# emanuele-artioli/elvis

Hardware: AMD Instinct MI355X
Metric: restored 1080p frames/sec, SinSR 4x path (ELVIS v2 Downsample) (higher is better)
Workload: dtype f16; 1 GPU; 30-frame 1920x1080 synthetic clip per GPU, ELVIS v2 Downsample (SinSR 4x), block 8, levels 0-3, weights seed 0 (random init), quantize=True; frames_per_gpu=30, parallelism=single GPU, gn_fused_into_conv=True, frames_per_invocation=15

## Files before the change

### elvis_amd/_lib.py

```python
from __future__ import annotations

import ctypes as C
import os
import threading
from typing import Optional

HERE = os.path.dirname(os.path.abspath(__file__))
LIBPATH = os.environ.get("ELVIS_AMD_LIB") or os.path.join(HERE, "lib", "libelvis_amd.so")

F32, F16 = 0, 1
ROUND_CV2, ROUND_HALF_UP = 0, 1
SSIM_LUMA, SSIM_CHANNELS = 0, 1
SSIM_REFLECT, SSIM_VALID = 0, 1
SSIM_PAD_AUTO = -1

_lock = threading.Lock()
_lib: Optional[C.CDLL] = None

vp, i32, f32, i64, f64 = C.c_void_p, C.c_int, C.c_float, C.c_longlong, C.c_double


class ConvDesc(C.Structure):
    _fields_ = [(n, C.c_int) for n in (
        "dtype", "n", "h", "w", "cin", "cin_pitch", "cin2", "cin2_pitch", "cout", "cout_pitch",
        "ksize", "stride", "pad_before", "upsample", "ho", "wo", "act", "prologue", "subpixel")]


SIGNATURES = {
    "elvis_abi_version": [],
    "elvis_last_error": [],
    "elvis_last_launch": [],
    "elvis_recompose_u8": [vp, vp, vp, vp, vp, i32, i32, i32, i32, i32, i32, i32, i32, i32, vp],
    "elvis_area_downscale_u8": [vp, vp, i32, i32, i32, i32, i32, i32, vp],
    "elvis_blend_u8": [vp, vp, vp, vp, i32, i32, i32, i32, i32, i32, i32, f32, vp],
    "elvis_select_levels_u8": [vp, vp, i32, vp, vp, i32, i32, i32, i32, i32, i32, i32, vp],
    "elvis_tile_accumulate_f32": [vp, vp, vp, vp, vp, vp, i32, i32, i32, i32, i32, i32, i32, f32, vp],
    "elvis_tile_normalize_u8": [vp, vp, vp, i32, i32, i32, vp],
    "elvis_sse_u8": [vp, vp, vp, vp, vp, i32, i32, i32, i32, vp],
    "elvis_block_ssim_u8": [vp, vp, vp, vp, i32, i32, i32, i32, i32, vp],
    "elvis_mask_bbox_u8": [vp, vp, i32, i32, i32, vp],
    "elvis_apply_mask_u8": [vp, vp, vp, i32, i32, i32, i32, i32, vp],
    "elvis_ssim_workspace_bytes": [i32, i32, i32, i32],
    "elvis_ssim_mean_f64": [vp, vp, vp, vp, vp, vp, vp, i32, i32, i32, i32, i32, i32, f64, f64, f64, i32, f64, vp],
    "elvis_u8_to_float": [vp, vp, i32, i32, i32, i32, i32, f32, f32, i32, i32, vp],
    "elvis_float_to_u8": [vp, i32, vp, vp, i32, i32, i32, i32, f32, f32, i32, i32, vp],
    "elvis_conv_packed_weight_bytes": [C.POINTER(ConvDesc)],
    "elvis_conv_pack_weights": [C.POINTER(ConvDesc), vp, vp, vp],
    "elvis_conv2d": [C.POINTER(ConvDesc), vp, vp, vp, vp, vp, i32, vp, vp, vp, vp, vp],
    "elvis_conv_stats_tiles": [C.POINTER(ConvDesc)],
    "elvis_conv_kernel_name": [C.POINTER(ConvDesc), C.c_char_p, C.c_size_t],
    "elvis_conv_kernel_name_for_call": [C.POINTER(ConvDesc), i32, i32, C.c_char_p, C.c_size_t],
    "elvis_conv_x3_eligible": [C.POINTER(ConvDesc)],
    "elvis_conv_debug_set": [C.c_char_p, i32],
    "elvis_gn_partials_to_sums": [vp, i32, i32, i32, vp, i32, i32, vp],
    "elvis_groupnorm_workspace_floats": [i32, i32, i32, i32],
    "elvis_groupnorm_sums": [vp, i32, i32, i32, i32, i32, vp, i32, i32, vp, vp],
    "elvis_groupnorm_affine": [vp, vp, vp, vp, vp, vp, vp, i32, i32, i32, i32, f32, vp],
    "elvis_affine_act": [vp, vp, i32, i32, i32, i32, i32, i32, vp, vp, i32, vp],
    "elvis_layernorm": [vp, vp, i32, i64, i32, i32, i32, vp, vp, f32, vp],
    "elvis_swin_packed_bytes": [i32, i32, i32],
    "elvis_swin_pack_weights": [vp, vp, vp, i32, i32, i32, vp],
    "elvis_swin_mlp": [vp, vp, vp, vp, vp, vp, vp, i64, i32, i32, i32, i32, f32, vp],
    "elvis_swin_ln_linear": [vp, vp, vp, vp, vp, vp, i64, i32, i32, i32, i32, f32, vp],
    "elvis_swin_pack_proj_mlp": [vp, vp, vp, vp, i32, i32, vp],
    "elvis_swin_proj_mlp": [vp, vp, vp, vp, vp, vp, vp, vp, vp, i64, i32, i32, i32, i32, i32, f32, vp],
    "elvis_window_attention": [vp, vp, i32, i32, i32, i32, i32, i32, i32, i32, i32, i32, vp, f32, vp],
    "elvis_bicubic_upsample": [vp, vp, i32, i32, i32, i32, i32, i32, i32, i32, vp],
    "elvis_vq_nearest": [vp, vp, vp, i32, i64, i32, i32, i32, vp, i32, vp],
    "elvis_pad_reflect_axpy": [vp, vp, i32, i32, i32, i32, i32, i32, i32, i32, i32, i32, f32, vp, f32, vp],
    "elvis_crop_copy": [vp, vp, i32, i32, i32, i32, i32, i32, i32, i32, i32, vp],
    "elvis_convert_act": [vp, i32, vp, i32, i64, i32, vp],
    "elvis_degrade_downsample_u8": [vp, vp, vp, i32, i32, i32, i32, i32, i32, i32, vp],
    "elvis_degrade_gaussian_u8": [vp, vp, vp, i32, i32, i32, i32, i32, i32, i32, f32, f32, f32, vp],
    "elvis_degrade_dct_u8": [vp, vp, vp, vp, vp, i32, i32, i32, i32, i32, i32, i32, vp],
    "elvis_degrade_scale_u8": [vp, vp, vp, i32, i32, i32, i32, i32, i32, i32, vp, vp, vp, i32, vp],
    "elvis_degrade_gaussian_fx_u8": [vp, vp, vp, i32, i32, i32, i32, i32, i32, i32, i32, i32, i32, vp],
    "elvis_rgb_to_i420_u8": [vp, vp, i32, i32, i32, i32, vp],
    "elvis_i420_to_rgb_u8": [vp, vp, i32, i32, i32, i32, vp],
    "elvis_classical_lanczos_u8": [vp, vp, vp, i32, i32, i32, i32, i32, i32, i32, vp, vp],
    "elvis_classical_unsharp_u8": [vp, vp, vp, i32, i32, i32, i32, i32, i32, i32, i32, vp, vp, i32, vp],
    "elvis_temporal_blend_u8": [vp, vp, i32, i64, f64, f64, vp],
# ... 19 lines not shown
    "elvis_rrdb_packed_weight_bytes": [i32, i32],
    "elvis_rrdb_pack_weights": [vp, i32, i32, i32, i32, vp],
    "elvis_rrdb_conv3x3": [vp, i32, vp, vp, vp, i32, i32, vp, i32, vp, i32, i32, i32, i32, i32, i32, i32, i32, f32, f32, i32, i32, vp],
    "elvis_rrdb_input_u8": [vp, vp, i32, i32, i32, i32, i32, vp],
    "elvis_dcnv2": [vp, vp, vp, vp, vp, i32, i32, i32, i32, i32, i32, i32, i32, i32, i32, i32, i32, vp],
    "elvis_temporal_stack": [vp, vp, i32, i32, i32, i32, i32, i32, i32, i32, vp],
    "elvis_plane_merge": [vp, vp, vp, i32, i32, i32, i32, i32, i32, vp],
}


def lib() -> C.CDLL:
    global _lib
    if _lib is not None:
        return _lib
    with _lock:
        if _lib is not None:
            return _lib
        if not os.path.exists(LIBPATH):
            raise RuntimeError(
                f"libelvis_amd.so not found at {LIBPATH}. Build it with `python -m elvis_amd._build` "
                "(needs hipcc). There is no CPU fallback for the restoration path.")
        import torch
        try:
            handle = C.CDLL(LIBPATH)
        except OSError as exc:
            raise RuntimeError(f"failed to load {LIBPATH}: {exc}") from exc
        for name, argtypes in SIGNATURES.items():
            fn = getattr(handle, name)
            fn.argtypes = argtypes
            fn.restype = C.c_int
        handle.elvis_last_error.restype = C.c_char_p
        handle.elvis_last_launch.restype = C.c_char_p
        handle.elvis_conv_packed_weight_bytes.restype = C.c_size_t
        handle.elvis_groupnorm_workspace_floats.restype = C.c_size_t
        handle.elvis_swin_packed_bytes.restype = C.c_size_t
        handle.elvis_ssim_workspace_bytes.restype = C.c_size_t
        handle.elvis_inpaint_workspace_bytes.restype = C.c_size_t
        handle.elvis_lpips_distance_workspace_bytes.restype = C.c_size_t
        handle.elvis_rrdb_packed_weight_bytes.restype = C.c_size_t
        if handle.elvis_abi_version() != 1:
            raise RuntimeError("libelvis_amd.so ABI version mismatch")
        _lib = handle
    return _lib


def check(rc: int, device=None) -> None:
    if rc == 0:
        return
    msg = lib().elvis_last_error().decode("utf-8", "replace")
    if rc == -1:
        raise ValueError(msg)
    label = str(device) if device is not None else "unknown device"
    raise RuntimeError(f"elvis_amd kernel failed on {label}: {msg}")


def ptr(t) -> int:
    return 0 if t is None else t.data_ptr()


def stream_handle(device=None) -> int:
    import torch
    return torch.cuda.current_stream(device).cuda_stream


def require_gpu(device) -> None:
    import torch
# ... 24 lines not shown
```

### elvis_amd/csrc/conv.hip

```cpp
#include "conv_kernels.inc"
#include "conv_ws.inc"
#include <string.h>

__attribute__((visibility("hidden"))) int elvis_conv_launch_f32_(const void* conv_args, int halo, int tco, int id, hipStream_t stream, void* query);
__attribute__((visibility("hidden"))) int elvis_conv_pack_x3p_(const float* w_oihw, void* packed, int cout, int ctot, int nkc, int n_co_tiles,
                                                              int tco, int taps, hipStream_t stream);

#include <atomic>
static std::atomic<int> g_no_halo{0};
static bool no_halo() { return g_no_halo.load(std::memory_order_relaxed) > 0; }
extern "C" int elvis_conv_debug_set(const char* key, int value) {
    ELVIS_REQUIRE(key, "elvis_conv_debug_set: null key");
    if (!strcmp(key, "no_halo")) { g_no_halo.store(value, std::memory_order_relaxed); return ELVIS_OK; }
    ELVIS_REQUIRE(false, "elvis_conv_debug_set: unknown key '%s'", key);
}

static void conv_geom(const elvis_conv_desc* d, int* nkc1, int* nkc, int* co_pad) {
    int kc = kc_of(d);
    *nkc1 = (d->cin + kc - 1) / kc;
    *nkc = *nkc1 + (d->cin2 > 0 ? (d->cin2 + kc - 1) / kc : 0);
    TileCfg t = choose_tile(d->cout);
    *co_pad = ((d->cout + t.tco - 1) / t.tco) * t.tco;
}

extern "C" size_t elvis_conv_packed_weight_bytes(const elvis_conv_desc* d) {
    if (!d || d->cin <= 0 || d->cout <= 0) return 0;
    int nkc1, nkc, co_pad;
    conv_geom(d, &nkc1, &nkc, &co_pad);
    return (size_t)d->ksize * d->ksize * nkc * co_pad * (x3_planar_fmt(d) ? 128 : 64);
}

extern "C" int elvis_conv_pack_weights(const elvis_conv_desc* d, const float* w_oihw, void* packed,
                                       elvis_stream_t stream) {
    int rc = validate(d);
    if (rc) return rc;
    ELVIS_REQUIRE(w_oihw && packed, "elvis_conv_pack_weights: null pointer");
    int nkc1, nkc, co_pad;
    conv_geom(d, &nkc1, &nkc, &co_pad);
    if (x3_planar_fmt(d)) {
        const int tco = choose_tile(d->cout).tco;
        return elvis_conv_pack_x3p_(w_oihw, packed, d->cout, d->cin + d->cin2, nkc, co_pad / tco, tco, d->ksize * d->ksize, (hipStream_t)stream);
    }
    int KC = kc_elems(d->dtype);
    long long total = (long long)d->ksize * d->ksize * nkc * co_pad * KC;
    int grid = (int)((total + 255) / 256);
    int ctot = d->cin + d->cin2;
// ... 71 lines not shown
    int rc = conv_walk(d, path, a, nullptr, &pick);
    if (rc) return rc;
    a.tiles_x = ((subpix ? d->w : d->wo) + HALO_TX - 1) / HALO_TX;
    a.tiles_y = pick.ty > 0 ? ((subpix ? d->h : d->ho) + pick.ty - 1) / pick.ty : 0;
    a.strip = HALO_STRIP < a.tiles_x ? HALO_STRIP : 0;
    a.strip_full = a.strip > 0 ? a.tiles_x / a.strip : 0;
    return ELVIS_OK;
}

extern "C" int elvis_conv_stats_tiles(const elvis_conv_desc* d) {
    if (!d || !halo_eligible(d)) return 0;
    ConvArgs a{};
    ConvPick pick{};
    if (conv_plan(d, ConvPath::HALO, a, pick)) return 0;
    return d->n * a.tiles_y * a.tiles_x;
}

extern "C" int elvis_conv_kernel_name_for_call(const elvis_conv_desc* d, int has_residual, int has_stats, char* buf, size_t n) {
    int rc = validate(d);
    if (rc) return rc;
    ELVIS_REQUIRE(buf && n > 0, "elvis_conv_kernel_name: null buffer");
    ConvArgs a{};
    ConvPick pick{};
    rc = conv_plan(d, conv_path(d, has_residual != 0, has_stats != 0), a, pick);
    if (rc) return rc;
    snprintf(buf, n, "%s", pick.name);
    return ELVIS_OK;
}

extern "C" int elvis_conv_kernel_name(const elvis_conv_desc* d, char* buf, size_t n) {
    return elvis_conv_kernel_name_for_call(d, 0, 0, buf, n);
}

extern "C" int elvis_conv2d(const elvis_conv_desc* d, const void* x, const void* x2, const void* w_packed,
                            const float* bias, const void* residual, int residual_pitch, const float* pa,
                            const float* pb, void* out, float* stats, elvis_stream_t stream) {
    int rc = validate(d);
    if (rc) return rc;
    ELVIS_REQUIRE(x && w_packed && out, "elvis_conv2d: null pointer");
    ELVIS_REQUIRE(d->cin2 == 0 || x2, "elvis_conv2d: cin2 > 0 but x2 is null");
    ELVIS_REQUIRE(!d->prologue || (pa && pb), "elvis_conv2d: prologue requested without pa/pb");
    ELVIS_REQUIRE(d->dtype != ELVIS_F32X3 || x3_eligible(d),
                  "elvis_conv2d: this shape has no compensated-f16 kernel (elvis_conv_x3_eligible): run it as ELVIS_F32");
    ELVIS_REQUIRE(!residual || residual_pitch >= d->cout, "elvis_conv2d: bad residual pitch");
    ELVIS_REQUIRE(((uintptr_t)x | (uintptr_t)(x2 ? x2 : x) | (uintptr_t)w_packed | (uintptr_t)out) % 16 == 0,
                  "elvis_conv2d: pointers must be 16-byte aligned");
    const ConvPath path = conv_path(d, residual != nullptr, stats != nullptr);
    ELVIS_REQUIRE(path != ConvPath::IGEMM || !stats, "elvis_conv2d: fused statistics need a 3x3/stride-1 conv with cout >= 64 (query elvis_conv_stats_tiles)");
    ELVIS_REQUIRE(path == ConvPath::IGEMM || (long long)d->n * d->h * d->w < 0x7fffffffLL, "conv: input too large for 32-bit pixel indices");
    ConvArgs a{};
    ConvPick pick{};
    rc = conv_plan(d, path, a, pick);
    if (rc) return rc;
    a.x = x; a.x2 = x2; a.w = w_packed; a.bias = bias; a.res = residual; a.pa = pa; a.pb = pb; a.out = out;
    a.res_pitch = residual_pitch; a.stats = stats;
    return conv_walk(d, path, a, (hipStream_t)stream, nullptr);
}
```

### elvis_amd/csrc/conv_kernels.inc

```
#pragma once
#include "common.h"

#ifndef ELVIS_CONV_HOOKS
#define ELVIS_STAGE(x) x
#define ELVIS_STAGE_W(x) x
#define ELVIS_STAGE_H(x) x
#define ELVIS_SETPRIO(x)
#define ELVIS_BARRIER() __syncthreads()
#define ELVIS_HOOK_SKIP_STORE(tv)
#define ELVIS_HOOK_STAMP_BEGIN
#define ELVIS_HOOK_STAMP_LOOP
#define ELVIS_HOOK_STAMP_EPILOGUE
#define ELVIS_HOOK_STAMP_END
#endif

namespace {

struct ConvArgs {
    const void* x;
    const void* x2;
    const void* w;
    const float* bias;
    const void* res;
    const float* pa;
    const float* pb;
    void* out;
    int n, h, w_in;
    int cin, cin_pitch, cin2, cin2_pitch;
    int cout, cout_pitch, res_pitch;
    int ksize, stride, pad, upsample;
    int ho, wo;
    int act, prologue;
    int nkc;
    int nkc1;
    int co_pad;
    long long M;
    int n_co_tiles;
    long long n_px_tiles;
    int two, tall;
    float* stats;
    int tiles_x, tiles_y;
    int sub, par_a, par_b;
    int ostr, pad2y, pad2x;
    int s2d, istr, nkc_c, wfull;
    int strip;
    int strip_full;
    int x3;
};

struct ConvPick {
    const char* name;
    int ty;
    int set(const char* name_, int ty_) { name = name_; ty = ty_; return ELVIS_OK; }
};
constexpr const char* tf(bool b) { return b ? "true" : "false"; }

template <typename T> struct Frag;
template <> struct Frag<half_t> { typedef half8 type; };
template <> struct Frag<float> { typedef float4v type; };

__device__ __forceinline__ void mma_tile(float4v& acc, const half8& a, const half8& b) {
    acc = __builtin_amdgcn_mfma_f32_16x16x32_f16(a, b, acc, 0, 0, 0);
}
__device__ __forceinline__ void mma_tile(float4v& acc, const float4v& a, const float4v& b) {
    acc = __builtin_amdgcn_mfma_f32_16x16x4f32(a[0], b[0], acc, 0, 0, 0);
    acc = __builtin_amdgcn_mfma_f32_16x16x4f32(a[1], b[1], acc, 0, 0, 0);
    acc = __builtin_amdgcn_mfma_f32_16x16x4f32(a[2], b[2], acc, 0, 0, 0);
    acc = __builtin_amdgcn_mfma_f32_16x16x4f32(a[3], b[3], acc, 0, 0, 0);
}

__device__ __forceinline__ unsigned x3_pair(float v) {
    const half_t h = (half_t)v;
    const half_t l = (half_t)(v - (float)h);
    return (unsigned)__builtin_bit_cast(unsigned short, h) | ((unsigned)__builtin_bit_cast(unsigned short, l) << 16);
}
__device__ __forceinline__ uint4 x3_pair4(uint4 v) {
    return make_uint4(x3_pair(__builtin_bit_cast(float, v.x)), x3_pair(__builtin_bit_cast(float, v.y)),
                      x3_pair(__builtin_bit_cast(float, v.z)), x3_pair(__builtin_bit_cast(float, v.w)));
}
template <bool X3> __device__ __forceinline__ void mma_tile_x(float4v& acc, const half8& a, const half8& b) { mma_tile(acc, a, b); }
// ... 389 lines not shown
    unsigned bid = blockIdx.x;
    {
        const unsigned q = nblk >> 3, r = nblk & 7u;
        const unsigned xcd = bid & 7u, idx = bid >> 3;
        bid = (xcd < r ? xcd * (q + 1) : r * (q + 1) + (xcd - r) * q) + idx;
    }
    int co_tile = 0;
    unsigned t = bid;
    if (p.n_co_tiles > 1) {
        t = bid / (unsigned)p.n_co_tiles;
        co_tile = (int)(bid - t * (unsigned)p.n_co_tiles);
    }
    int tx, ty, nimg;
    if (p.strip > 0) {
        const unsigned per_img = (unsigned)p.tiles_x * (unsigned)p.tiles_y;
        const unsigned ni = t / per_img;
        unsigned r = t - ni * per_img;
        const unsigned full = (unsigned)p.strip_full, strip_tiles = (unsigned)p.strip * (unsigned)p.tiles_y;
        unsigned s = r / strip_tiles;
        unsigned sw = (unsigned)p.strip;
        if (s >= full) { s = full; sw = (unsigned)p.tiles_x - full * (unsigned)p.strip; }
        r -= s * strip_tiles;
        const unsigned y = r / sw;
        nimg = (int)ni;
        ty = (int)y;
        tx = (int)(s * (unsigned)p.strip + (r - y * sw));
    } else {
        const unsigned row = t / (unsigned)p.tiles_x;
        tx = (int)(t - row * (unsigned)p.tiles_x);
        const unsigned ni = row / (unsigned)p.tiles_y;
        ty = (int)(row - ni * (unsigned)p.tiles_y);
        nimg = (int)ni;
    }
    const int oy0 = ty * TY, ox0 = tx * TX, co0 = co_tile * TCO;

    const int tid = threadIdx.x, lane = tid & 63, wave = tid >> 6;
    ELVIS_HOOK_STAMP_BEGIN
    const int w_co = wave / NW_PX, w_px = wave % NW_PX;
    const int lh = p.upsample ? p.h * 2 : p.h, lw = p.upsample ? p.w_in * 2 : p.w_in;

    const int pad_y = KS == 2 ? p.pad2y : KS / 2, pad_x = KS == 2 ? p.pad2x : KS / 2;
    int h_src[H_PER];
    unsigned h_ok = 0;
#pragma unroll
    for (int i = 0; i < H_PER; ++i) {
        int chunk = tid + i * NT;
        int pix = chunk >> 2;
        int hy = pix / HX, hx = pix - hy * HX;
        int gy = oy0 + hy - pad_y, gx = ox0 + hx - pad_x;
        bool ok = chunk < HCH && gy >= 0 && gy < lh && gx >= 0 && gx < lw;
        int sy = p.upsample ? (gy >> 1) : gy, sx = p.upsample ? (gx >> 1) : gx;
        h_src[i] = ok ? ((nimg * p.h + sy) * p.istr * p.w_in + sx) * p.istr : 0;
        h_ok |= (ok ? 1u : 0u) << i;
    }
    const bool halo_inside = oy0 - pad_y >= 0 && oy0 - pad_y + HY <= lh && ox0 - pad_x >= 0 && ox0 - pad_x + HX <= lw &&
                             (p.cin % KC) == 0 && (p.cin2 % KC) == 0 && p.cin_pitch >= p.nkc1 * KC && !(KS == 2 && p.s2d);
    const int q4 = tid & 3;
    const int nkc = p.nkc;
    const int nrows = nkc * KS;

    constexpr int HA = (H_PER + 1) / 2;
    uint4 hreg[H_PER];

    int wl_off[W_PER];
#pragma unroll
    for (int i = 0; i < W_PER; ++i) {
        int chunk = tid + i * NT;
        wl_off[i] = lds_row_off(chunk >> 2, chunk & 3);
    }

    auto chunk_c0 = [&](int kc, int& pixoff) -> int {
        pixoff = 0;
        if (KS == 2 && p.s2d) {
            const int ph = kc / p.nkc_c;
            pixoff = (ph >> 1) * p.wfull + (ph & 1);
            return (kc - ph * p.nkc_c) * KC + q4 * VEC;
        }
        return (kc >= p.nkc1 ? kc - p.nkc1 : kc) * KC + q4 * VEC;
    };
    auto halo_load = [&](int kc, int i0, int i1, bool live = true) {
        const bool second = kc >= p.nkc1;
        const char* xsrc = (const char*)(second ? p.x2 : p.x);
        const int pitch = second ? p.cin2_pitch : p.cin_pitch;
        int pixoff;
        const int c0 = chunk_c0(kc, pixoff);
        const int c0c = c0 < pitch ? c0 : 0;
        const long long lv = live ? (long long)sizeof(T) : 0;
#pragma unroll
        for (int i = i0; i < i1; ++i)
            hreg[i] = *reinterpret_cast<const uint4*>(xsrc + ((long long)(h_src[i] + pixoff) * pitch + c0c) * lv);
    };
    auto halo_store = [&](int kc, int buf, int i0, int i1) {
        const bool second = kc >= p.nkc1;
        const int pitch = second ? p.cin2_pitch : p.cin_pitch;
        int pixoff_;
        const int c0 = chunk_c0(kc, pixoff_);
        const bool ch_ok = c0 < pitch;
        char* dst = halo + buf * HALO_BYTES;
        float la[VEC], lb[VEC];
        if (PRO) {
            const float* tp = ptab + (kc * 4 + q4) * 2 * VEC;
#pragma unroll
            for (int e = 0; e < VEC; e += 4) {
                float4v a4 = *reinterpret_cast<const float4v*>(tp + e);
                float4v b4 = *reinterpret_cast<const float4v*>(tp + VEC + e);
#pragma unroll
                for (int k = 0; k < 4; ++k) { la[e + k] = a4[k]; lb[e + k] = b4[k]; }
            }
        }
#pragma unroll
        for (int i = i0; i < i1; ++i) {
            uint4 v = hreg[i];
            if constexpr (PSC) {
                const float K = -1.4426950408889634f;
                v.x = prologue_dword_f16(v.x, la[0], la[1], lb[0], lb[1], K);
                v.y = prologue_dword_f16(v.y, la[2], la[3], lb[2], lb[3], K);
                v.z = prologue_dword_f16(v.z, la[4], la[5], lb[4], lb[5], K);
                v.w = prologue_dword_f16(v.w, la[6], la[7], lb[6], lb[7], K);
            } else if (PRO) {
                v = prologue_apply<T>(v, la, lb);
            }
            if constexpr (X3) v = x3_pair4(v);
            if (!halo_inside) {
                const bool keep = ch_ok && ((h_ok >> i) & 1u);
                v.x = keep ? v.x : 0u; v.y = keep ? v.y : 0u; v.z = keep ? v.z : 0u; v.w = keep ? v.w : 0u;
            }
            int chunk = tid + i * NT;
            if ((i + 1) * NT <= HCH || chunk < HCH)
                *reinterpret_cast<uint4*>(dst + lds_row_off(chunk >> 2, chunk & 3)) = v;
        }
    };
    auto halo_act = [&](int kc, int slot, int half) {
        constexpr int HV = VEC / 2;
        const float* tp = ptab + (kc * 4 + q4) * 2 * VEC + half * HV;
        float a[HV], b[HV];
#pragma unroll
        for (int e = 0; e < HV; e += 2) {
            float2 a2 = *reinterpret_cast<const float2*>(tp + e);
            float2 b2 = *reinterpret_cast<const float2*>(tp + VEC + e);
            a[e] = a2.x; a[e + 1] = a2.y; b[e] = b2.x; b[e + 1] = b2.y;
        }
        uint2 v = half ? make_uint2(hreg[slot].z, hreg[slot].w) : make_uint2(hreg[slot].x, hreg[slot].y);
        v = prologue_apply_half(v, a, b, T());
        if (half) { hreg[slot].z = v.x; hreg[slot].w = v.y; } else { hreg[slot].x = v.x; hreg[slot].y = v.y; }
    };
    auto halo_write = [&](int kc, int buf, int slot) {
        const bool second = kc >= p.nkc1;
        const int pitch = second ? p.cin2_pitch : p.cin_pitch;
        int pixoff_;
        const int c0 = chunk_c0(kc, pixoff_);
        const bool keep = c0 < pitch && ((h_ok >> slot) & 1u);
        uint4 v = hreg[slot];
        if constexpr (X3) v = x3_pair4(v);
        v.x = keep ? v.x : 0u; v.y = keep ? v.y : 0u; v.z = keep ? v.z : 0u; v.w = keep ? v.w : 0u;
        int chunk = tid + slot * NT;
        if ((slot + 1) * NT <= HCH || chunk < HCH)
            *reinterpret_cast<uint4*>(halo + buf * HALO_BYTES + lds_row_off(chunk >> 2, chunk & 3)) = v;
    };
    static_assert(W_PER <= 2, "weight staging holds at most two 16-byte chunks per thread per tap");
    constexpr bool W_FULL0 = W_CHUNKS >= NT, W_FULL1 = W_PER == 2 && W_CHUNKS >= 2 * NT;
    const bool w_ok0 = W_FULL0 || tid < W_CHUNKS, w_ok1 = W_PER == 2 && (W_FULL1 || tid + NT < W_CHUNKS);
    uint4 wr00 = {}, wr01 = {}, wr10 = {}, wr11 = {}, wr20 = {}, wr21 = {};
// ... 227 lines not shown
#pragma unroll
        for (int r = 0; r < 4; ++r)
#pragma unroll
            for (int e = 0; e < 2; ++e) {
                int carry = ((pp0 & 3) + r) >> 2;
                int bit = ((pp0 >> 2) & 1) ^ carry ^ e;
                bb[r][e] = pp0 * 64 + ((lq ^ (bit << 1)) << 4);
            }
        const int a_off = HALO_BYTES + w_co * WCO * 1024 + lane_off;
        ELVIS_HOOK_STAMP_LOOP
        for (int kc = 0; kc < nkc; ++kc) {
            if (kc + G1_NST - 2 < nkc) asm volatile("s_waitcnt vmcnt(%0)" :: "n"((G1_NST - 2) * L) : "memory");
            else asm volatile("s_waitcnt vmcnt(0)" ::: "memory");
            __syncthreads();
            if (kc + G1_NST - 1 < nkc) g1_issue(kc + G1_NST - 1);
            const int sb = (kc % G1_NST) * STAGE;
            frag_t fa[WCO];
#pragma unroll
            for (int i = 0; i < WCO; ++i) fa[i] = lds_frag<frag_t>(smem + sb + a_off + i * 1024);
#pragma unroll
            for (int j = 0; j < WPX; ++j) {
                const int C = (j >> 1) * HX + (j & 1) * 16;
                frag_t fb = lds_frag<frag_t>(smem + sb + bb[C & 3][(C >> 2) & 1] + C * 64);
#pragma unroll
                for (int i = 0; i < WCO; ++i) mma_tile_x<X3>(acc[i][j], fa[i], fb);
            }
        }
        __syncthreads();
    } else {
    if constexpr (!EARLY && !G1) {
        halo_load(0, 0, H_PER);
        if constexpr (WDMA) w_glds(0, 0); else w_load(0);
    }
    if (PRO) {
        const int ctot = p.cin + p.cin2;
        for (int t2 = tid; t2 < nkc * 4 * VEC; t2 += NT) {
            int kc = t2 / (4 * VEC), r = t2 - kc * 4 * VEC;
            bool second = kc >= p.nkc1;
            int cl = (second ? kc - p.nkc1 : kc) * KC + r;
            bool in = cl < (second ? p.cin2 : p.cin);
            long long g = (long long)nimg * ctot + (second ? p.cin : 0) + (in ? cl : 0);
            int q = r / VEC, e = r - q * VEC;
            const float psc = PSC ? -1.4426950408889634f : 1.0f;
            ptab[(kc * 4 + q) * 2 * VEC + e] = in ? psc * p.pa[g] : 0.0f;
            ptab[(kc * 4 + q) * 2 * VEC + VEC + e] = in ? psc * p.pb[g] : 0.0f;
        }
        __syncthreads();
    }
    halo_store(0, 0, 0, H_PER);
    res_convert();
    if constexpr (WDMA) {
        w_glds_wait();
    } else {
        w_store(0);
        w_load(1);
    }
    __syncthreads();

    ELVIS_HOOK_STAMP_LOOP
    const int pp0 = (w_px * ROWS) * HX + lr;
    int bb[4][2];
#pragma unroll
    for (int r = 0; r < 4; ++r)
#pragma unroll
        for (int e = 0; e < 2; ++e) {
            int carry = ((pp0 & 3) + r) >> 2;
            int bit = ((pp0 >> 2) & 1) ^ carry ^ e;
// ... 595 lines not shown
```

### elvis_amd/ops.py

```python
from __future__ import annotations

import ctypes as C
from dataclasses import dataclass
from typing import Optional

import numpy as np
import torch

from . import _lib as L
from ._lib import ConvDesc, check, lib, ptr


def _s(t: torch.Tensor) -> int:
    return torch.cuda.current_stream(t.device).cuda_stream


def pitch_for(c: int) -> int:
    return (c + 7) // 8 * 8


@dataclass
class Act:
    t: torch.Tensor
    c: int
# ... 193 lines not shown
                bias = torch.cat([bias, bias.new_zeros(self.cout_k - cout)], 0)
        self.x3 = bool(_X3_DEFAULT if x3 is None else x3) and dtype == torch.float32
        d = ConvDesc()
        d.dtype = L.dtype_code(dtype)
        d.n = d.h = d.w = d.ho = d.wo = 1
        d.cin, d.cin_pitch, d.cin2, d.cin2_pitch = cin, pitch_for(cin), cin2, pitch_for(cin2) if cin2 else 0
        d.cout, d.cout_pitch = self.cout_k, pitch_for(cout)
        d.ksize, d.stride = kh, 1
        if kh == 2:
            d.subpixel, d.ho, d.wo = 1, 2, 2
        nbytes = lib().elvis_conv_packed_weight_bytes(C.byref(d))
        w_dev = weight_oihw.to(device=device, dtype=torch.float32).contiguous()
        self.packed = torch.empty(nbytes, dtype=torch.uint8, device=device)
        check(lib().elvis_conv_pack_weights(C.byref(d), ptr(w_dev), ptr(self.packed), _s(self.packed)), device)
        self.packed_x3 = None
        if self.x3:
            d.dtype = F32X3_CODE
            nbytes = lib().elvis_conv_packed_weight_bytes(C.byref(d))
            self.packed_x3 = torch.empty(nbytes, dtype=torch.uint8, device=device)
            check(lib().elvis_conv_pack_weights(C.byref(d), ptr(w_dev), ptr(self.packed_x3), _s(self.packed_x3)), device)
        torch.cuda.current_stream(device).synchronize()
        self.bias = None if bias is None else bias.to(device=device, dtype=torch.float32).contiguous()

    def weights_for(self, d) -> torch.Tensor:
        if self.packed_x3 is not None:
            keep, d.dtype = d.dtype, F32X3_CODE
            if lib().elvis_conv_x3_eligible(C.byref(d)):
                return self.packed_x3
            d.dtype = keep
        return self.packed

    def __call__(self, x: Act, x2: Optional[Act] = None, *, stride=1, pad=None, upsample=False, act=0,
                 residual: Optional[Act] = None, prologue=None, out: Optional[Act] = None, ho=None, wo=None,
                 want_stats: bool = False) -> Act:
        if x.c != self.cin or (x2.c if x2 is not None else 0) != self.cin2:
            raise ValueError(f"conv: expected inputs with {self.cin}+{self.cin2} channels, got {x.c}+{x2.c if x2 else 0}")
        for t in (x, x2, residual):
            if t is not None and t.t.dtype != self.dtype:
                raise ValueError(f"conv: weights are packed for {self.dtype}, got a {t.t.dtype} tensor")
        d = ConvDesc()
        d.dtype = x.dtype_code
        d.n, d.h, d.w = x.n, x.h, x.w
        d.cin, d.cin_pitch = x.c, x.pitch
        d.cin2, d.cin2_pitch = (x2.c, x2.pitch) if x2 is not None else (0, 0)
        d.ksize, d.stride, d.upsample, d.act = self.ksize, stride, int(upsample), act
        d.pad_before = (self.ksize // 2) if pad is None else pad
        lh, lw = (x.h * 2, x.w * 2) if upsample else (x.h, x.w)
        if ho is None:
            ho = (lh + 2 * d.pad_before - self.ksize) // stride + 1
            wo = (lw + 2 * d.pad_before - self.ksize) // stride + 1
        d.ho, d.wo = ho, wo
        if out is None:
            out = new_act(x.n, ho, wo, self.cout, x.t.dtype, x.t.device, zero=False)
        d.cout, d.cout_pitch = self.cout_k, out.pitch
        pa = pb = None
        if prologue is not None:
            pa, pb = prologue
            d.prologue = 1
        stats = None
        packed = self.weights_for(d)
        tiles = lib().elvis_conv_stats_tiles(C.byref(d))
        if want_stats and tiles > 0:
            stats = torch.empty((tiles, self.cout_k, 2), dtype=torch.float32, device=x.t.device)
        out.stats = stats
        prof = CONV_PROFILER
        if prof is not None:
            e0, e1 = torch.cuda.Event(enable_timing=True), torch.cuda.Event(enable_timing=True)
            e0.record()
        check(lib().elvis_conv2d(C.byref(d), ptr(x.t), ptr(x2.t) if x2 is not None else 0, ptr(packed),
                                 ptr(self.bias), ptr(residual.t) if residual is not None else 0,
                                 residual.pitch if residual is not None else 0, ptr(pa), ptr(pb), ptr(out.t),
                                 ptr(stats), _s(x.t)), x.t.device)
        if prof is not None:
            e1.record()
            flops = 2.0 * self.ksize * self.ksize * (self.cin + self.cin2) * self.cout * x.n * ho * wo
            name = conv_kernel_name(d, residual=residual is not None, stats=stats is not None)
            if name.startswith("conv3x3_ws_kernel") and residual is None and KERNEL_PROFILER is not None:
                nbytes = float(self.cin + self.cin2 + self.cout) * x.t.element_size() * x.n * ho * wo
                KERNEL_PROFILER.append((name, "hbm", nbytes, e0, e1))
            else:
                prof.append((name, flops, e0, e1))
            if CONV_SHAPES is not None:
                CONV_SHAPES.append((x.n, x.h, x.w, self.cin + self.cin2, self.cout, self.ksize, stride,
                                    prologue is not None, residual is not None))
        if stats is not None and self.cout_k != self.cout:
            out.stats = stats[:, :self.cout].contiguous()
        return out


CONV_PROFILER = None
CONV_SHAPES = None
KERNEL_PROFILER = None


class _Timed:
    def __init__(self, name, bound, work):
        self.rec = (name, bound, work) if KERNEL_PROFILER is not None else None

    def __enter__(self):
        if self.rec:
            self.e0, self.e1 = torch.cuda.Event(enable_timing=True), torch.cuda.Event(enable_timing=True)
            self.e0.record()

    def __exit__(self, *exc):
        if self.rec and KERNEL_PROFILER is not None:
# ... 315 lines not shown
```

### include/elvis_amd.h

```cpp
#ifndef ELVIS_AMD_H
#define ELVIS_AMD_H

#include <stddef.h>
#include <stdint.h>

#ifdef __cplusplus
extern "C" {
#endif

#define ELVIS_ABI_VERSION 1

#define ELVIS_OK 0
#define ELVIS_E_INVALID (-1)
#define ELVIS_E_RUNTIME (-2)
#define ELVIS_E_UNSUPPORTED (-3)

#define ELVIS_F32 0
#define ELVIS_F16 1
#define ELVIS_F32X3 2

#define ELVIS_ROUND_CV2 0
#define ELVIS_ROUND_HALF_UP 1

typedef void* elvis_stream_t;
// ... 52 lines not shown
int elvis_u8_to_float(const uint8_t* src, void* dst, int dtype, int n, int h, int w, int pitch,
                      float scale, float bias, int swap_rb, int div255, elvis_stream_t stream);

int elvis_float_to_u8(const void* src, int dtype, uint8_t* dst, float* f32_out, int n, int h, int w,
                      int pitch, float scale, float bias, int mode, int swap_rb, elvis_stream_t stream);


typedef struct elvis_conv_desc {
    int dtype;
    int n, h, w;
    int cin, cin_pitch;
    int cin2, cin2_pitch;
    int cout, cout_pitch;
    int ksize;
    int stride;
    int pad_before;
    int upsample;
    int ho, wo;
    int act;
    int prologue;
    int subpixel;
} elvis_conv_desc;
#define ELVIS_CONV_S2D 5

size_t elvis_conv_packed_weight_bytes(const elvis_conv_desc* d);

int elvis_conv_pack_weights(const elvis_conv_desc* d, const float* w_oihw, void* packed,
                            elvis_stream_t stream);

int elvis_conv2d(const elvis_conv_desc* d, const void* x, const void* x2, const void* w_packed,
                 const float* bias, const void* residual, int residual_pitch, const float* pa,
                 const float* pb, void* out, float* stats, elvis_stream_t stream);

int elvis_conv_stats_tiles(const elvis_conv_desc* d);

int elvis_conv_kernel_name(const elvis_conv_desc* d, char* buf, size_t n);

int elvis_conv_kernel_name_for_call(const elvis_conv_desc* d, int has_residual, int has_stats, char* buf, size_t n);

int elvis_conv_debug_set(const char* key, int value);

int elvis_conv_x3_eligible(const elvis_conv_desc* d);

int elvis_gn_partials_to_sums(const float* partials, int tiles_per_image, int n, int c, double* sums,
                              int sums_ctot, int sums_coff, elvis_stream_t stream);

size_t elvis_groupnorm_workspace_floats(int dtype, int n, int hw, int c);
int elvis_groupnorm_sums(const void* x, int dtype, int n, int hw, int c, int pitch, double* sums,
                         int sums_ctot, int sums_coff, float* workspace, elvis_stream_t stream);

int elvis_groupnorm_affine(const double* sums, const float* gamma, const float* beta, const float* scale,
                           const float* shift, float* pa, float* pb, int n, int hw, int c, int groups,
                           float eps, elvis_stream_t stream);


int elvis_affine_act(const void* x, void* y, int dtype, int n, int hw, int c, int pitch_in,
                     int pitch_out, const float* pa, const float* pb, int act, elvis_stream_t stream);

int elvis_layernorm(const void* x, void* y, int dtype, long long tokens, int c, int pitch_in,
                    int pitch_out, const float* gamma, const float* beta, float eps, elvis_stream_t stream);

size_t elvis_swin_packed_bytes(int c, int n1, int mode);
int elvis_swin_pack_weights(const float* w1, const float* w2, void* packed, int c, int n1, int mlp, elvis_stream_t stream);
int elvis_swin_mlp(const void* x, void* out, const void* packed, const float* b1, const float* b2, const float* gamma,
                   const float* beta, long long tokens, int c, int hidden, int x_pitch, int out_pitch, float eps,
                   elvis_stream_t stream);
// ... 153 lines not shown
```

Baseline: 32.16 frames/s.

## Split prologue conv: first co-tile writes activated input, rest reuse it

For f16 3x3 convs with a fused GroupNorm/SiLU prologue and several 128-wide output-channel tiles, the conv now runs in two launches. The first launch computes only the first co-tile and also writes the prologue-activated input to a planar scratch buffer. The second launch covers the remaining co-tiles and reads that scratch with the prologue skipped. This avoids recomputing the prologue transcendentals once per co-tile, at the cost of an extra launch, a scratch allocation per call and extra HBM traffic to write and reread the activated input.

Measured after the change: 32.13 frames/s. Within noise of the previous version (-0.1%).

```diff
diff --git a/elvis_amd/_lib.py b/elvis_amd/_lib.py
--- a/elvis_amd/_lib.py
+++ b/elvis_amd/_lib.py
@@ -47,6 +47,8 @@
     "elvis_conv_packed_weight_bytes": [C.POINTER(ConvDesc)],
     "elvis_conv_pack_weights": [C.POINTER(ConvDesc), vp, vp, vp],
     "elvis_conv2d": [C.POINTER(ConvDesc), vp, vp, vp, vp, vp, i32, vp, vp, vp, vp, vp],
+    "elvis_conv_prologue_scratch_bytes": [C.POINTER(ConvDesc)],
+    "elvis_conv2d_scratch": [C.POINTER(ConvDesc), vp, vp, vp, vp, vp, i32, vp, vp, vp, vp, vp, vp, C.c_size_t],
     "elvis_conv_stats_tiles": [C.POINTER(ConvDesc)],
     "elvis_conv_kernel_name": [C.POINTER(ConvDesc), C.c_char_p, C.c_size_t],
     "elvis_conv_kernel_name_for_call": [C.POINTER(ConvDesc), i32, i32, C.c_char_p, C.c_size_t],
@@ -132,6 +134,7 @@
         handle.elvis_last_error.restype = C.c_char_p
         handle.elvis_last_launch.restype = C.c_char_p
         handle.elvis_conv_packed_weight_bytes.restype = C.c_size_t
+        handle.elvis_conv_prologue_scratch_bytes.restype = C.c_size_t
         handle.elvis_groupnorm_workspace_floats.restype = C.c_size_t
         handle.elvis_swin_packed_bytes.restype = C.c_size_t
         handle.elvis_ssim_workspace_bytes.restype = C.c_size_t
diff --git a/elvis_amd/csrc/conv.hip b/elvis_amd/csrc/conv.hip
--- a/elvis_amd/csrc/conv.hip
+++ b/elvis_amd/csrc/conv.hip
@@ -7,11 +7,15 @@
                                                               int tco, int taps, hipStream_t stream);
 
 #include <atomic>
+#include <atomic>
 static std::atomic<int> g_no_halo{0};
+static std::atomic<int> g_split_min_tiles{0}, g_split_min_px_tiles{0};
 static bool no_halo() { return g_no_halo.load(std::memory_order_relaxed) > 0; }
 extern "C" int elvis_conv_debug_set(const char* key, int value) {
     ELVIS_REQUIRE(key, "elvis_conv_debug_set: null key");
     if (!strcmp(key, "no_halo")) { g_no_halo.store(value, std::memory_order_relaxed); return ELVIS_OK; }
+    if (!strcmp(key, "split_min_tiles")) { g_split_min_tiles.store(value, std::memory_order_relaxed); return ELVIS_OK; }
+    if (!strcmp(key, "split_min_px_tiles")) { g_split_min_px_tiles.store(value, std::memory_order_relaxed); return ELVIS_OK; }
     ELVIS_REQUIRE(false, "elvis_conv_debug_set: unknown key '%s'", key);
 }
 
@@ -149,9 +153,34 @@
     return elvis_conv_kernel_name_for_call(d, 0, 0, buf, n);
 }
 
+constexpr int SPLIT_MIN_TILES = 4, SPLIT_MIN_PX_TILES = 500;
+static bool conv_split_ok(const elvis_conv_desc* d) {
+    if (d->dtype != ELVIS_F16 || d->ksize != 3 || d->stride != 1 || d->upsample || !d->prologue) return false;
+    if (no_halo() || !halo_eligible(d) || !halo_two(d)) return false;
+    if ((long long)d->n * d->h * d->w * 64 >= (1LL << 32)) return false;
+    if (choose_tile(d->cout).tco != 128) return false;
+    const int dbg_t = g_split_min_tiles.load(std::memory_order_relaxed), dbg_p = g_split_min_px_tiles.load(std::memory_order_relaxed);
+    const long long px_tiles = (long long)d->n * ((d->h + HALO_TY2 - 1) / HALO_TY2) * ((d->w + HALO_TX - 1) / HALO_TX);
+    return d->cout / 128 >= (dbg_t > 0 ? dbg_t : SPLIT_MIN_TILES) && d->cout / 128 >= 2 &&
+           px_tiles >= (dbg_p > 0 ? dbg_p : SPLIT_MIN_PX_TILES);
+}
+static size_t conv_split_plane_bytes(const elvis_conv_desc* d) { return (size_t)d->n * d->h * d->w * 64; }
+
+extern "C" size_t elvis_conv_prologue_scratch_bytes(const elvis_conv_desc* d) {
+    if (!d || validate(d) || !conv_split_ok(d)) return 0;
+    return conv_split_plane_bytes(d) * conv_nkc32(d);
+}
+
 extern "C" int elvis_conv2d(const elvis_conv_desc* d, const void* x, const void* x2, const void* w_packed,
                             const float* bias, const void* residual, int residual_pitch, const float* pa,
                             const float* pb, void* out, float* stats, elvis_stream_t stream) {
+    return elvis_conv2d_scratch(d, x, x2, w_packed, bias, residual, residual_pitch, pa, pb, out, stats, stream, nullptr, 0);
+}
+
+extern "C" int elvis_conv2d_scratch(const elvis_conv_desc* d, const void* x, const void* x2, const void* w_packed,
+                                    const float* bias, const void* residual, int residual_pitch, const float* pa,
+                                    const float* pb, void* out, float* stats, elvis_stream_t stream, void* scratch,
+                                    size_t scratch_bytes) {
     int rc = validate(d);
     if (rc) return rc;
     ELVIS_REQUIRE(x && w_packed && out, "elvis_conv2d: null pointer");
@@ -171,5 +200,18 @@
     if (rc) return rc;
     a.x = x; a.x2 = x2; a.w = w_packed; a.bias = bias; a.res = residual; a.pa = pa; a.pb = pb; a.out = out;
     a.res_pitch = residual_pitch; a.stats = stats;
+    if (scratch && path == ConvPath::HALO && conv_split_ok(d)) {
+        ELVIS_REQUIRE((uintptr_t)scratch % 16 == 0 && scratch_bytes >= elvis_conv_prologue_scratch_bytes(d),
+                      "elvis_conv2d_scratch: scratch must be 16-byte aligned and hold elvis_conv_prologue_scratch_bytes(d) = %zu bytes (got %zu)",
+                      elvis_conv_prologue_scratch_bytes(d), scratch_bytes);
+        const int tiles = a.n_co_tiles;
+        a.act_out = scratch;
+        a.act_plane = (long long)conv_split_plane_bytes(d);
+        a.n_co_tiles = 1;
+        rc = conv_walk(d, path, a, (hipStream_t)stream, nullptr);
+        if (rc) return rc;
+        a.x = scratch; a.act_out = nullptr; a.act_in = 1;
+        a.co_first = 1; a.n_co_tiles = tiles - 1;
+    }
     return conv_walk(d, path, a, (hipStream_t)stream, nullptr);
 }
diff --git a/elvis_amd/csrc/conv_kernels.inc b/elvis_amd/csrc/conv_kernels.inc
--- a/elvis_amd/csrc/conv_kernels.inc
+++ b/elvis_amd/csrc/conv_kernels.inc
@@ -46,6 +46,10 @@
     int strip;
     int strip_full;
     int x3;
+    void* act_out;
+    long long act_plane;
+    int act_in;
+    int co_first;
 };
 
 struct ConvPick {
@@ -501,6 +505,10 @@
         ty = (int)(row - ni * (unsigned)p.tiles_y);
         nimg = (int)ni;
     }
+    constexpr bool SPLIT = PSC && KS == 3 && !X3 && TCO == 128;
+    if constexpr (SPLIT) co_tile += p.co_first;
+    const bool act_in = SPLIT && p.act_in != 0;
+    const bool act_out = SPLIT && p.act_out != nullptr;
     const int oy0 = ty * TY, ox0 = tx * TX, co0 = co_tile * TCO;
 
     const int tid = threadIdx.x, lane = tid & 63, wave = tid >> 6;
@@ -521,9 +529,14 @@
         int sy = p.upsample ? (gy >> 1) : gy, sx = p.upsample ? (gx >> 1) : gx;
         h_src[i] = ok ? ((nimg * p.h + sy) * p.istr * p.w_in + sx) * p.istr : 0;
         h_ok |= (ok ? 1u : 0u) << i;
+        if constexpr (SPLIT) {
+            static_assert(H_PER <= 16, "h_ok holds two bits per staged slot");
+            const bool own = ok && hy >= 1 && hy <= TY && hx >= 1 && hx <= TX;
+            h_ok |= (own ? 1u : 0u) << (16 + i);
+        }
     }
     const bool halo_inside = oy0 - pad_y >= 0 && oy0 - pad_y + HY <= lh && ox0 - pad_x >= 0 && ox0 - pad_x + HX <= lw &&
-                             (p.cin % KC) == 0 && (p.cin2 % KC) == 0 && p.cin_pitch >= p.nkc1 * KC && !(KS == 2 && p.s2d);
+                             (act_in || ((p.cin % KC) == 0 && (p.cin2 % KC) == 0 && p.cin_pitch >= p.nkc1 * KC)) && !(KS == 2 && p.s2d);
     const int q4 = tid & 3;
     const int nkc = p.nkc;
     const int nrows = nkc * KS;
@@ -550,10 +563,17 @@
     auto halo_load = [&](int kc, int i0, int i1, bool live = true) {
         const bool second = kc >= p.nkc1;
         const char* xsrc = (const char*)(second ? p.x2 : p.x);
-        const int pitch = second ? p.cin2_pitch : p.cin_pitch;
+        int pitch = second ? p.cin2_pitch : p.cin_pitch;
         int pixoff;
         const int c0 = chunk_c0(kc, pixoff);
-        const int c0c = c0 < pitch ? c0 : 0;
+        int c0c = c0 < pitch ? c0 : 0;
+        if constexpr (SPLIT) {
+            if (act_in) {
+                xsrc = (const char*)p.x + kc * p.act_plane;
+                pitch = KC;
+                c0c = q4 * VEC;
+            }
+        }
         const long long lv = live ? (long long)sizeof(T) : 0;
 #pragma unroll
         for (int i = i0; i < i1; ++i)
@@ -564,39 +584,58 @@
         const int pitch = second ? p.cin2_pitch : p.cin_pitch;
         int pixoff_;
         const int c0 = chunk_c0(kc, pixoff_);
-        const bool ch_ok = c0 < pitch;
+        const bool ch_ok = act_in || c0 < pitch;
         char* dst = halo + buf * HALO_BYTES;
-        float la[VEC], lb[VEC];
-        if (PRO) {
-            const float* tp = ptab + (kc * 4 + q4) * 2 * VEC;
-#pragma unroll
-            for (int e = 0; e < VEC; e += 4) {
-                float4v a4 = *reinterpret_cast<const float4v*>(tp + e);
-                float4v b4 = *reinterpret_cast<const float4v*>(tp + VEC + e);
-#pragma unroll
-                for (int k = 0; k < 4; ++k) { la[e + k] = a4[k]; lb[e + k] = b4[k]; }
-            }
-        }
-#pragma unroll
-        for (int i = i0; i < i1; ++i) {
-            uint4 v = hreg[i];
-            if constexpr (PSC) {
-                const float K = -1.4426950408889634f;
-                v.x = prologue_dword_f16(v.x, la[0], la[1], lb[0], lb[1], K);
-                v.y = prologue_dword_f16(v.y, la[2], la[3], lb[2], lb[3], K);
-                v.z = prologue_dword_f16(v.z, la[4], la[5], lb[4], lb[5], K);
-                v.w = prologue_dword_f16(v.w, la[6], la[7], lb[6], lb[7], K);
-            } else if (PRO) {
-                v = prologue_apply<T>(v, la, lb);
-            }
-            if constexpr (X3) v = x3_pair4(v);
-            if (!halo_inside) {
-                const bool keep = ch_ok && ((h_ok >> i) & 1u);
-                v.x = keep ? v.x : 0u; v.y = keep ? v.y : 0u; v.z = keep ? v.z : 0u; v.w = keep ? v.w : 0u;
-            }
-            int chunk = tid + i * NT;
-            if ((i + 1) * NT <= HCH || chunk < HCH)
-                *reinterpret_cast<uint4*>(dst + lds_row_off(chunk >> 2, chunk & 3)) = v;
+        auto stage = [&](auto pro_) {
+            constexpr bool PRO_ = decltype(pro_)::value;
+            float la[VEC], lb[VEC];
+            if (PRO_) {
+                const float* tp = ptab + (kc * 4 + q4) * 2 * VEC;
+#pragma unroll
+                for (int e = 0; e < VEC; e += 4) {
+                    float4v a4 = *reinterpret_cast<const float4v*>(tp + e);
+                    float4v b4 = *reinterpret_cast<const float4v*>(tp + VEC + e);
+#pragma unroll
+                    for (int k = 0; k < 4; ++k) { la[e + k] = a4[k]; lb[e + k] = b4[k]; }
+                }
+            }
+#pragma unroll
+            for (int i = i0; i < i1; ++i) {
+                uint4 v = hreg[i];
+                if constexpr (PSC && PRO_) {
+                    const float K = -1.4426950408889634f;
+                    v.x = prologue_dword_f16(v.x, la[0], la[1], lb[0], lb[1], K);
+                    v.y = prologue_dword_f16(v.y, la[2], la[3], lb[2], lb[3], K);
+                    v.z = prologue_dword_f16(v.z, la[4], la[5], lb[4], lb[5], K);
+                    v.w = prologue_dword_f16(v.w, la[6], la[7], lb[6], lb[7], K);
+                } else if (PRO_) {
+                    v = prologue_apply<T>(v, la, lb);
+                }
+                if constexpr (X3) v = x3_pair4(v);
+                if (!halo_inside) {
+                    const bool keep = ch_ok && ((h_ok >> i) & 1u);
+                    v.x = keep ? v.x : 0u; v.y = keep ? v.y : 0u; v.z = keep ? v.z : 0u; v.w = keep ? v.w : 0u;
+                }
+                int chunk = tid + i * NT;
+                if ((i + 1) * NT <= HCH || chunk < HCH)
+                    *reinterpret_cast<uint4*>(dst + lds_row_off(chunk >> 2, chunk & 3)) = v;
+                if constexpr (SPLIT && PRO_) hreg[i] = v;
+            }
+            if constexpr (SPLIT && PRO_) {
+                if (act_out) {
+                    char* const plane = (char*)p.act_out + kc * p.act_plane;
+#pragma unroll
+                    for (int i = i0; i < i1; ++i)
+                        if ((h_ok >> (16 + i)) & 1u)
+                            *reinterpret_cast<uint4*>(plane + ((unsigned)h_src[i] * 64u + (unsigned)q4 * 16u)) = hreg[i];
+                }
+            }
+        };
+        if constexpr (SPLIT) {
+            if (act_in) stage(std::false_type{});
+            else stage(std::true_type{});
+        } else {
+            stage(std::integral_constant<bool, PRO>{});
         }
     };
     auto halo_act = [&](int kc, int slot, int half) {
@@ -890,7 +929,7 @@
         halo_load(0, 0, H_PER);
         if constexpr (WDMA) w_glds(0, 0); else w_load(0);
     }
-    if (PRO) {
+    if (PRO && !act_in) {
         const int ctot = p.cin + p.cin2;
         for (int t2 = tid; t2 < nkc * 4 * VEC; t2 += NT) {
             int kc = t2 / (4 * VEC), r = t2 - kc * 4 * VEC;
diff --git a/elvis_amd/ops.py b/elvis_amd/ops.py
--- a/elvis_amd/ops.py
+++ b/elvis_amd/ops.py
@@ -249,7 +249,7 @@
 
     def __call__(self, x: Act, x2: Optional[Act] = None, *, stride=1, pad=None, upsample=False, act=0,
                  residual: Optional[Act] = None, prologue=None, out: Optional[Act] = None, ho=None, wo=None,
-                 want_stats: bool = False) -> Act:
+                 want_stats: bool = False, scratch=True) -> Act:
         if x.c != self.cin or (x2.c if x2 is not None else 0) != self.cin2:
             raise ValueError(f"conv: expected inputs with {self.cin}+{self.cin2} channels, got {x.c}+{x2.c if x2 else 0}")
         for t in (x, x2, residual):
@@ -284,10 +284,16 @@
         if prof is not None:
             e0, e1 = torch.cuda.Event(enable_timing=True), torch.cuda.Event(enable_timing=True)
             e0.record()
-        check(lib().elvis_conv2d(C.byref(d), ptr(x.t), ptr(x2.t) if x2 is not None else 0, ptr(packed),
-                                 ptr(self.bias), ptr(residual.t) if residual is not None else 0,
-                                 residual.pitch if residual is not None else 0, ptr(pa), ptr(pb), ptr(out.t),
-                                 ptr(stats), _s(x.t)), x.t.device)
+        sbuf, sbytes = None, 0
+        if prologue is not None and scratch is not False:
+            sbytes = lib().elvis_conv_prologue_scratch_bytes(C.byref(d))
+            if sbytes:
+                sbuf = scratch if isinstance(scratch, torch.Tensor) else torch.empty(sbytes, dtype=torch.uint8, device=x.t.device)
+                sbytes = sbuf.numel()
+        check(lib().elvis_conv2d_scratch(C.byref(d), ptr(x.t), ptr(x2.t) if x2 is not None else 0, ptr(packed),
+                                         ptr(self.bias), ptr(residual.t) if residual is not None else 0,
+                                         residual.pitch if residual is not None else 0, ptr(pa), ptr(pb), ptr(out.t),
+                                         ptr(stats), _s(x.t), ptr(sbuf), sbytes), x.t.device)
         if prof is not None:
             e1.record()
             flops = 2.0 * self.ksize * self.ksize * (self.cin + self.cin2) * self.cout * x.n * ho * wo
diff --git a/include/elvis_amd.h b/include/elvis_amd.h
--- a/include/elvis_amd.h
+++ b/include/elvis_amd.h
@@ -108,6 +108,13 @@
                  const float* bias, const void* residual, int residual_pitch, const float* pa,
                  const float* pb, void* out, float* stats, elvis_stream_t stream);
 
+size_t elvis_conv_prologue_scratch_bytes(const elvis_conv_desc* d);
+
+int elvis_conv2d_scratch(const elvis_conv_desc* d, const void* x, const void* x2, const void* w_packed,
+                         const float* bias, const void* residual, int residual_pitch, const float* pa,
+                         const float* pb, void* out, float* stats, elvis_stream_t stream, void* scratch,
+                         size_t scratch_bytes);
+
 int elvis_conv_stats_tiles(const elvis_conv_desc* d);
 
 int elvis_conv_kernel_name(const elvis_conv_desc* d, char* buf, size_t n);
```
